# FordyceLab/magnify

Measured on NVIDIA B200. Metric: roi_pixels_per_sec, higher is better.
Workload: dtype u16

## Files before the change

### include/magnify_b200.h

```cpp
#ifndef MAGNIFY_B200_H
#define MAGNIFY_B200_H

#include <stdint.h>

#ifdef __cplusplus
extern "C" {
#endif

#define MGB_ABI_VERSION 12

#define MGB_OK 0
#define MGB_EINVAL (-1)
#define MGB_EALIGN (-2)
#define MGB_EUNSUPPORTED (-3)
#define MGB_EIO (-4)
#define MGB_EFORMAT (-5)

#define MGB_U8 0
#define MGB_U16 1
#define MGB_F32 2
#define MGB_F64 3

int mgb_abi_version(void);
const char* mgb_error_string(int code);
// ... 23 lines not shown
                             const double* bias, const double* maxima, void* stream);
int mgb_flatfield_apply_generic(const void* tiles, void* out, int dtype, int64_t C, int64_t P,
                                int64_t HW, int K, const double* flat, const double* dark,
                                const double* maxima, void* stream);

int mgb_copy2d_async(void* dst, int64_t dst_pitch_bytes, const void* src, int64_t src_pitch_bytes,
                     int64_t width_bytes, int64_t rows, int kind, void* stream);

int mgb_bounding_boxes(const double* x, const double* y, int64_t n, int L, int64_t W, int64_t H,
                       int32_t* boxes, int32_t* rel, void* stream);

int mgb_set_tma_enabled(int enabled);
int mgb_set_gather_loader(int loader);

int mgb_roi_gather(const void* image, int64_t image_pitch, int64_t C, int64_t T, int64_t H, int64_t W,
                   int itemsize, const int32_t* boxes, const int32_t* order, int64_t M, int L, void* roi,
                   void* stream);
int mgb_roi_gather_stats_u16(const uint16_t* image, int64_t image_pitch, int64_t C, int64_t T, int64_t H,
                             int64_t W, const int32_t* boxes, const int32_t* order, const int32_t* mask_t,
                             int64_t Tm, const uint8_t* fg, const uint8_t* bg, int64_t M, int L,
                             uint16_t* roi, double* stats, int want_median, int fg_count_max,
                             int bg_count_max, int* host_median_done, void* stream);
int mgb_mask_count_max(const uint8_t* fg, const uint8_t* bg, int64_t n_masks, int64_t mask_len,
                       int32_t* counts, void* stream);
int mgb_roi_gather_stats_peers_u16(const uint16_t* image, int64_t image_pitch, int64_t C, int64_t T,
                                   int64_t H, int64_t W, const int32_t* boxes, const int32_t* order, const int32_t* mask_t,
                                   int64_t Tm, const uint8_t* fg, const uint8_t* bg, int64_t M, int L,
                                   uint16_t* roi, const uint64_t* host_peer_stats, int n_peers,
                                   int want_median, int fg_count_max, int bg_count_max,
                                   int* host_median_done, void* stream);
int mgb_roi_stats_u16(const uint16_t* roi, int64_t M, int64_t C, int64_t T, int L,
                      const int32_t* mask_t, int64_t Tm, const uint8_t* fg, const uint8_t* bg,
                      double* stats, void* stream);
int mgb_roi_median_u16(const uint16_t* roi, int64_t M, int64_t C, int64_t T, int L,
                       const int32_t* mask_t, int64_t Tm, const uint8_t* mask, double* median,
                       int64_t median_stride, void* stream);

int mgb_roi_stats_f32(const float* roi, int64_t M, int64_t C, int64_t T, int L, const int32_t* mask_t, int64_t Tm,
                      const uint8_t* fg, const uint8_t* bg, double* stats, void* stream);
int mgb_roi_median_f32(const float* roi, int64_t M, int64_t C, int64_t T, int L, const int32_t* mask_t, int64_t Tm,
                       const uint8_t* mask, double* median, int64_t median_stride, void* stream);

int mgb_chip_masks(const int32_t* rel, const int32_t* r_fg, int r_inner, int r_outer, int64_t M,
                   int L, uint8_t* fg, uint8_t* bg, int32_t* counts, void* stream);

int mgb_mask_perimeters(const uint8_t* masks, int64_t M, int L, double* perimeter, void* stream);

int mgb_disc_halfwidths(int r, int32_t* host_hw);
int mgb_bead_labels(const int32_t* beads, int64_t M, int64_t H, int64_t W, const int32_t* hw,
                    int rmax, int32_t* labels, void* stream);
int mgb_bead_masks(const int32_t* labels, int64_t H, int64_t W, const int32_t* boxes, int64_t M,
                   int L, uint8_t* fg, uint8_t* bg, int32_t* counts, void* stream);

int mgb_to_uint8(const void* src, int dtype, int64_t B, int64_t n, uint8_t* dst, double* minmax, void* stream);
int mgb_edge_gradients_u8(const uint8_t* image, int64_t B, int64_t H, int64_t W, uint8_t* blurred, int16_t* dx,
                          int16_t* dy, void* stream);
int mgb_gradient_order_stats(const int16_t* dx, const int16_t* dy, int64_t B, int64_t n, const int64_t* host_ranks,
                             int n_ranks, int64_t* host_values, uint32_t* scratch, void* stream);
int mgb_canny(const int16_t* dx, const int16_t* dy, int64_t B, int64_t H, int64_t W, const int32_t* thresholds,
              uint8_t* edges, int* changed, int* host_sweeps, void* stream);

int mgb_edge_cell_lists(const uint8_t* edges, int64_t B, int64_t H, int64_t W, int grid_length, int64_t* counts,
                        int64_t* starts, uint32_t* coords, int64_t coords_capacity, int64_t* host_total, void* stream);
int mgb_sample_circles(const uint32_t* coords, const int64_t* starts, const int64_t* counts, int64_t B, int64_t H,
                       int64_t W, int grid_length, int64_t num_iter, float min_radius, float max_radius,
                       uint64_t seed, const uint32_t* randoms, float* raw, uint64_t* table, int64_t table_capacity,
// ... 30 lines not shown
```

### magnify_b200/_lib.py

```python
from __future__ import annotations

import ctypes
import os
from ctypes import c_char_p, c_int, c_int64, c_void_p, POINTER

_PKG_DIR = os.path.dirname(os.path.abspath(__file__))
LIB_PATH = os.path.join(_PKG_DIR, "libmagnify_b200.so")

MGB_U8, MGB_U16, MGB_F32, MGB_F64 = 0, 1, 2, 3
MGB_EINVAL, MGB_EALIGN, MGB_EUNSUPPORTED, MGB_EIO, MGB_EFORMAT = -1, -2, -3, -4, -5


class MagnifyB200Error(RuntimeError):
    def __init__(self, fn: str, code: int, text: str):
        super().__init__(f"{fn} failed with status {code}: {text}")
        self.fn, self.code = fn, code


_P = c_void_p
_I64 = c_int64
SIGNATURES = {
    "mgb_abi_version": [],
    "mgb_error_string": [c_int],
    "mgb_sm_count": [],
    "mgb_launch_count": [],
    "mgb_l2_persist": [_P, _P, _I64, ctypes.c_float],
    "mgb_set_tma_enabled": [c_int],
    "mgb_set_stitch_variant": [c_int],
    "mgb_set_gather_loader": [c_int],
    "mgb_stitch": [_P, _P, _I64, _I64, _I64, _I64, _I64, _I64, _I64, _I64, c_int, POINTER(c_int), _P],
    "mgb_flatfield_tilemax_u16": [_P, _I64, _I64, _I64, c_int, c_int, _P, _P],
    "mgb_flatfield_maxima": [_P, c_int, c_int, _I64, _P, _P, _P, _P],
    "mgb_flatfield_maxima_generic": [_P, c_int, _I64, _I64, _I64, c_int, _P, _P, _P, _P],
    "mgb_flatfield_tables": [_P, _P, c_int, _I64, _P, _P, _P, _P],
    "mgb_flatfield_stitch_u16": [_P, _P, _I64, _I64, _I64, _I64, _I64, _I64, _I64, _I64, c_int, _P, _P, _P, _P, _P, _P],
    "mgb_flatfield_apply_generic": [_P, _P, c_int, _I64, _I64, _I64, c_int, _P, _P, _P, _P],
    "mgb_copy2d_async": [_P, _I64, _P, _I64, _I64, _I64, c_int, _P],
    "mgb_bounding_boxes": [_P, _P, _I64, c_int, _I64, _I64, _P, _P, _P],
    "mgb_roi_gather": [_P, _I64, _I64, _I64, _I64, _I64, c_int, _P, _P, _I64, c_int, _P, _P],
    "mgb_roi_gather_stats_u16": [_P, _I64, _I64, _I64, _I64, _I64, _P, _P, _P, _I64, _P, _P, _I64, c_int, _P, _P,
                                 c_int, c_int, c_int, POINTER(c_int), _P],
    "mgb_mask_count_max": [_P, _P, _I64, _I64, _P, _P],
    "mgb_roi_gather_stats_peers_u16": [_P, _I64, _I64, _I64, _I64, _I64, _P, _P, _P, _I64, _P, _P, _I64, c_int, _P,
                                       POINTER(ctypes.c_uint64), c_int, c_int, c_int, c_int, POINTER(c_int), _P],
    "mgb_roi_stats_u16": [_P, _I64, _I64, _I64, c_int, _P, _I64, _P, _P, _P, _P],
    "mgb_roi_median_u16": [_P, _I64, _I64, _I64, c_int, _P, _I64, _P, _P, _I64, _P],
    "mgb_roi_stats_f32": [_P, _I64, _I64, _I64, c_int, _P, _I64, _P, _P, _P, _P],
    "mgb_roi_median_f32": [_P, _I64, _I64, _I64, c_int, _P, _I64, _P, _P, _I64, _P],
    "mgb_chip_masks": [_P, _P, c_int, c_int, _I64, c_int, _P, _P, _P, _P],
    "mgb_disc_halfwidths": [c_int, POINTER(ctypes.c_int32)],
    "mgb_bead_labels": [_P, _I64, _I64, _I64, _P, c_int, _P, _P],
    "mgb_bead_masks": [_P, _I64, _I64, _P, _I64, c_int, _P, _P, _P, _P],
    "mgb_mask_perimeters": [_P, _I64, c_int, _P, _P],
    "mgb_to_uint8": [_P, c_int, _I64, _I64, _P, _P, _P],
    "mgb_edge_gradients_u8": [_P, _I64, _I64, _I64, _P, _P, _P, _P],
    "mgb_gradient_order_stats": [_P, _P, _I64, _I64, POINTER(c_int64), c_int, POINTER(c_int64), _P, _P],
    "mgb_canny": [_P, _P, _I64, _I64, _I64, _P, _P, _P, POINTER(c_int), _P],
    "mgb_edge_cell_lists": [_P, _I64, _I64, _I64, c_int, _P, _P, _P, _I64, POINTER(c_int64), _P],
    "mgb_sample_circles": [_P, _P, _P, _I64, _I64, _I64, c_int, _I64, ctypes.c_float, ctypes.c_float, ctypes.c_uint64,
                           _P, _P, _P, _I64, _P, POINTER(c_int64), _P, _P],
    "mgb_gradient_angles": [_P, _P, _P, _I64, _P, _P],
    "mgb_circle_perimeter": [c_int, c_int, POINTER(ctypes.c_int32), c_int, POINTER(c_int)],
    "mgb_score_circles": [_P, _I64, _I64, _I64, _P, _P, c_int, c_int, _P, _P, _P, _P, _P],
    "mgb_order_circles": [_P, _P, _I64, _P, _P],
    "mgb_filter_neighbors_device": [_P, _I64, _I64, _I64, _I64, c_int, c_int, _P, _P, POINTER(c_int), _P],
    "mgb_filter_neighbors": [POINTER(ctypes.c_int32), _I64, c_int, POINTER(ctypes.c_uint8)],
    "mgb_tiff_open": [c_char_p, POINTER(c_void_p)],
    "mgb_tiff_close": [_P],
    "mgb_tiff_page_count": [_P, POINTER(c_int64)],
    "mgb_tiff_page_info": [_P, _I64, POINTER(c_int64)],
    "mgb_tiff_description": [_P, _I64, c_char_p, _I64],
    "mgb_tiff_read_pages": [_P, POINTER(c_int64), _I64, _P, _I64, c_int],
    "mgb_tiff_write": [c_char_p, _P, _I64, _I64, _I64, c_int, c_int, c_int, c_char_p, c_int],
    "mgb_tiff_read_files": [POINTER(c_char_p), _I64, _I64, _I64, _I64, c_int, _P, _I64, c_int],
}
_SPECIAL_RESTYPE = {"mgb_error_string": c_char_p, "mgb_launch_count": c_int64}
_NO_STATUS = {"mgb_abi_version", "mgb_error_string", "mgb_sm_count", "mgb_launch_count", "mgb_set_tma_enabled", "mgb_set_stitch_variant", "mgb_set_gather_loader"}

# ... 38 lines not shown
```

### magnify_b200/csrc/roi.cu

```cuda
#include "common.cuh"

namespace mgb {

__device__ __forceinline__ void box_1d(long long c, int L, long long size, long long* lo) {
  long long a = c - L / 2;
  long long b = c + (L + 1) / 2;
  if (a < 0) { b -= a; a = 0; }
  if (b > size) { a -= b - size; }
  *lo = a;
}

__global__ void __launch_bounds__(kThreads)
bounding_boxes_kernel(const double* __restrict__ x, const double* __restrict__ y, int64_t n, int L,
                      int64_t W, int64_t H, int32_t* __restrict__ boxes, int32_t* __restrict__ rel) {
  const int64_t i = (int64_t)blockIdx.x * blockDim.x + threadIdx.x;
  if (i >= n) return;
  const long long xr = __double2ll_rn(x[i]);
  const long long yr = __double2ll_rn(y[i]);
  long long top, left;
  box_1d(yr, L, H, &top);
  box_1d(xr, L, W, &left);
  boxes[2 * i] = (int32_t)top;
  boxes[2 * i + 1] = (int32_t)left;
  if (rel) {
// ... 312 lines not shown
    const float x = src[i];
    if (x != x) continue;
    if (fg[moff + i]) { v[0] += 1.0; v[2] += (double)x; }
    if (bg[moff + i]) { v[1] += 1.0; v[3] += (double)x; }
  }
#pragma unroll
  for (int k = 0; k < 4; ++k) {
    for (int o = 16; o > 0; o >>= 1) v[k] += __shfl_down_sync(0xffffffffu, v[k], o);
    if ((threadIdx.x & 31) == 0) red[k][threadIdx.x >> 5] = v[k];
  }
  __syncthreads();
  if (threadIdx.x == 0) {
    double s[4] = {0.0, 0.0, 0.0, 0.0};
    for (int w = 0; w < kThreads / 32; ++w)
      for (int k = 0; k < 4; ++k) s[k] += red[k][w];
    double* out = stats + n * kRec;
    out[0] = s[0]; out[1] = s[1]; out[2] = s[2]; out[3] = s[3];
    out[4] = s[2] / s[0];
    out[5] = s[3] / s[1];
    out[6] = out[7] = __longlong_as_double(0x7ff8000000000000LL);
  }
}

static uint32_t magic_for(uint32_t d) { return (uint32_t)((0x100000000ULL + d - 1) / d); }

int roi_gather_tma(const void* image, int64_t pitch, int64_t C, int64_t T, int64_t H, int64_t W, int itemsize,
                   const int32_t* boxes, const int32_t* order, const int32_t* mask_t, int64_t Tm, const uint8_t* fg,
                   const uint8_t* bg, int64_t M, int L, void* roi, double* stats, const uint64_t* host_peers,
                   int n_peers, cudaStream_t st);

int roi_gather_lists(const void* image, int64_t pitch, int64_t C, int64_t T, int64_t H, int64_t W,
                     const int32_t* boxes, const int32_t* order, const int32_t* mask_t, int64_t Tm, const uint8_t* fg,
                     const uint8_t* bg, int64_t M, int L, void* roi, double* stats, int want_median, int nf_max,
                     int nb_max, const uint64_t* host_peers, int n_peers, cudaStream_t st);

extern int g_gather_loader;
extern int g_gather_wpm;

static int g_tma_enabled = 1;

}

using namespace mgb;

template <typename TPix>
static int launch_roi_median(const TPix* roi, int64_t M, int64_t C, int64_t T, int L, const int32_t* mask_t, int64_t Tm,
                             const uint8_t* mask, double* median, int64_t stride, void* stream) {
  if (M < 0 || C < 0 || T < 0 || L <= 0 || stride < 1) return MGB_EINVAL;
  const int64_t n_roi = M * C * T;
  if (n_roi == 0) return MGB_OK;
  if (n_roi > INT32_MAX) return MGB_EUNSUPPORTED;
  if (!roi || !mask_t || !mask || !median || Tm <= 0) return MGB_EINVAL;
  cudaStream_t st = (cudaStream_t)stream;
  const int npt = (int)ceil_div((int64_t)L * L, kThreads);
#define MGB_MED(N) roi_median_kernel<N, TPix><<<(unsigned)n_roi, kThreads, 0, st>>>(roi, C, T, L, mask_t, Tm, mask, median, stride)
  if (npt <= 4) MGB_MED(4);
  else if (npt <= 10) MGB_MED(10);
  else if (npt <= 21) MGB_MED(21);
  else if (npt <= 40) MGB_MED(40);
  else if (npt <= 64) MGB_MED(64);
  else if (npt <= 100) MGB_MED(100);
  else roi_median_big_kernel<TPix><<<(unsigned)n_roi, kThreads, 0, st>>>(roi, C, T, L, mask_t, Tm, mask, median, stride);
#undef MGB_MED
  MGB_CUDA_LAUNCH_CHECK();
  return MGB_OK;
}

// ... 94 lines not shown
}

int mgb_roi_gather_stats_u16(const uint16_t* image, int64_t image_pitch, int64_t C, int64_t T, int64_t H,
                             int64_t W, const int32_t* boxes, const int32_t* order, const int32_t* mask_t, int64_t Tm,
                             const uint8_t* fg, const uint8_t* bg, int64_t M, int L,
                             uint16_t* roi, double* stats, int want_median, int fg_count_max, int bg_count_max,
                             int* host_median_done, void* stream) {
  if (host_median_done) *host_median_done = 0;
  if (!stats && M * C * T > 0) return MGB_EINVAL;
  return gather_common(image, image_pitch, C, T, H, W, 2, boxes, order, 0, mask_t, Tm, fg, bg, M, L, roi, stats,
                       (cudaStream_t)stream, nullptr, 0, want_median, fg_count_max, bg_count_max, host_median_done);
}

int mgb_roi_gather_stats_peers_u16(const uint16_t* image, int64_t image_pitch, int64_t C, int64_t T, int64_t H,
                                   int64_t W, const int32_t* boxes, const int32_t* order, const int32_t* mask_t,
                                   int64_t Tm, const uint8_t* fg, const uint8_t* bg, int64_t M, int L,
                                   uint16_t* roi, const uint64_t* host_peer_stats, int n_peers, int want_median,
                                   int fg_count_max, int bg_count_max, int* host_median_done, void* stream) {
  if (host_median_done) *host_median_done = 0;
  if (!host_peer_stats || n_peers < 1 || n_peers > 8) return MGB_EINVAL;
  if (M * C * T == 0) return MGB_OK;
  return gather_common(image, image_pitch, C, T, H, W, 2, boxes, order, 0, mask_t, Tm, fg, bg, M, L, roi,
                       reinterpret_cast<double*>(host_peer_stats[0]), (cudaStream_t)stream, host_peer_stats, n_peers,
                       want_median, fg_count_max, bg_count_max, host_median_done);
}

int mgb_roi_stats_u16(const uint16_t* roi, int64_t M, int64_t C, int64_t T, int L, const int32_t* mask_t,
                      int64_t Tm, const uint8_t* fg, const uint8_t* bg, double* stats, void* stream) {
  if (!stats && M * C * T > 0) return MGB_EINVAL;
  return gather_common(roi, 0, C, T, L, L, 2, nullptr, nullptr, C * T * (int64_t)L * L, mask_t, Tm, fg, bg, M, L, nullptr,
                       stats, (cudaStream_t)stream);
}

int mgb_roi_median_u16(const uint16_t* roi, int64_t M, int64_t C, int64_t T, int L,
                       const int32_t* mask_t, int64_t Tm, const uint8_t* mask, double* median,
                       int64_t median_stride, void* stream) {
  return launch_roi_median<uint16_t>(roi, M, C, T, L, mask_t, Tm, mask, median, median_stride, stream);
}

int mgb_roi_median_f32(const float* roi, int64_t M, int64_t C, int64_t T, int L, const int32_t* mask_t, int64_t Tm,
                       const uint8_t* mask, double* median, int64_t median_stride, void* stream) {
  return launch_roi_median<float>(roi, M, C, T, L, mask_t, Tm, mask, median, median_stride, stream);
}

int mgb_roi_stats_f32(const float* roi, int64_t M, int64_t C, int64_t T, int L, const int32_t* mask_t, int64_t Tm,
                      const uint8_t* fg, const uint8_t* bg, double* stats, void* stream) {
  if (M < 0 || C < 0 || T < 0 || L <= 0) return MGB_EINVAL;
  const int64_t n_roi = M * C * T;
  if (n_roi == 0) return MGB_OK;
  if (n_roi > INT32_MAX) return MGB_EUNSUPPORTED;
  if (!roi || !mask_t || !fg || !bg || !stats || Tm <= 0) return MGB_EINVAL;
  roi_stats_f32_kernel<<<(unsigned)n_roi, kThreads, 0, (cudaStream_t)stream>>>(roi, C, T, L, mask_t, Tm, fg, bg, stats);
  MGB_CUDA_LAUNCH_CHECK();
  return MGB_OK;
}

}
```

### magnify_b200/csrc/roi_lists.cu

```cuda
#include <algorithm>

#include "roi_stage.cuh"

namespace mgb {

constexpr int kNFL = 32;
constexpr int kNBL = 80;

__device__ __forceinline__ void stage_mask(const uint8_t* __restrict__ g, int n, uint8_t* s, int tid, int nth) {
  const uint32_t sa = smem_u32(s);
  if ((reinterpret_cast<uintptr_t>(g) & 15u) == 0) {
    const int nv = n >> 4;
    for (int i = tid; i < nv; i += nth)
      asm volatile("cp.async.ca.shared.global [%0], [%1], 16;" ::"r"(sa + 16u * i), "l"(g + 16 * i) : "memory");
    for (int i = (nv << 4) + tid; i < n; i += nth) s[i] = g[i];
  } else if ((reinterpret_cast<uintptr_t>(g) & 3u) == 0) {
    const int nv = n >> 2;
    for (int i = tid; i < nv; i += nth)
      asm volatile("cp.async.ca.shared.global [%0], [%1], 4;" ::"r"(sa + 4u * i), "l"(g + 4 * i) : "memory");
    for (int i = (nv << 2) + tid; i < n; i += nth) s[i] = g[i];
  } else {
    for (int i = tid; i < n; i += nth) s[i] = g[i];
  }
}
// ... 217 lines not shown
  const bool overflow = nf > (uint32_t)p.cap_f || nb > (uint32_t)p.cap_b;
  if (active && !overflow) {
    pad_list(fl, nf, p.cap_f, WPM ? lane : (int)threadIdx.x, WPM ? 32 : (int)blockDim.x);
    pad_list(bl, nb, p.cap_b, WPM ? lane : (int)threadIdx.x, WPM ? 32 : (int)blockDim.x);
  }
  __syncthreads();
  if (!active) return;
  const double cnt_fg = (double)nf, cnt_bg = (double)nb;
  const int GF = p.cap_f >> 8, GB = p.cap_b >> 8;
  const uint32_t pad_f = (uint32_t)p.cap_f - nf, pad_b = (uint32_t)p.cap_b - nb;

  const int nt = s_nt;
  const int n_items = nt * (int)p.C;

  constexpr int kV = VPL > 0 ? VPL : 1;
  const int nquads = (p.rows * p.wu) >> 2;

  uint8_t* my_stages = stages + (size_t)warp * p.n_stages * p.stage_bytes;
  const uint32_t my_stage0 = smem_u32(my_stages);
  const uint32_t my_bar0 = smem_u32(&bars[warp * 4]);
  uint32_t* my_hist = hists + (size_t)warp * kHistWords;
  const uint32_t tx_bytes = (uint32_t)(p.rows * p.wpu * 2);
  const int first = WPM ? 0 : part * nw + warp, step = WPM ? 1 : nparts * nw;

  struct Cursor { int i, c, k; };
  auto advance = [&](Cursor& cur, int by) {
    cur.i += by;
    cur.k += by;
    while (cur.k >= nt) { cur.k -= nt; ++cur.c; }
  };
  auto issue_tma = [&](const Cursor& cur, int s) {
    if (lane == 0) {
      const int64_t t = tlist[cur.k];
      const int32_t top = p.boxes[(m * p.T + t) * 2];
      const int32_t left = p.boxes[(m * p.T + t) * 2 + 1];
      const uint32_t bar = my_bar0 + s * 8;
      mbar_expect_tx(bar, tx_bytes);
      tma_load_3d(my_stage0 + s * p.stage_bytes, &tmap, bar, left & ~7, top, (int)(cur.c * p.T + t));
    }
  };

  Cursor ahead{0, 0, 0}, cur{0, 0, 0};
  if (nt > 0) { advance(ahead, first); advance(cur, first); }
  for (int s = 0; s < p.n_stages; ++s) {
    if (ahead.i < n_items) issue_tma(ahead, s);
    if (nt > 0) advance(ahead, step);
  }
  int s = 0;
  uint32_t parity = 0;
  for (; cur.i < n_items; advance(cur, step)) {
    const int64_t c = cur.c, t = tlist[cur.k];
    const int shift = p.boxes[(m * p.T + t) * 2 + 1] & 7;
    const int64_t n = (m * p.C + c) * p.T + t;
    const uint8_t* buf = my_stages + (size_t)s * p.stage_bytes;
    mbar_wait(my_bar0 + s * 8, parity);

    if (p.store) {
      uint16_t* dst = p.roi + n * (int64_t)p.rows * p.wu;
      uint32_t opaque = 0;
      asm volatile("" : "+r"(opaque));
      if constexpr (QPL > 0) {
        uint2* d2 = reinterpret_cast<uint2*>(dst);
        const uint32_t* s32 = reinterpret_cast<const uint32_t*>(buf);
        auto copy = [&](auto par) {
          constexpr int PAR = decltype(par)::value;
#pragma unroll
          for (int k = 0; k < QPL; ++k) {
            const int q = lane + 32 * k;
            if (q < nquads) {
              const uint32_t u = 4u * q + opaque;
              const uint32_t row = __umulhi(u, p.magic_wu), col = u - row * p.wu;
              const uint32_t oa = row * p.wpu + col + shift;
              const uint32_t ob = (col + 2 < (uint32_t)p.wu) ? oa + 2 : (row + 1) * p.wpu + shift;
              const uint32_t lo = load_pair<PAR>(s32, oa);
              const uint32_t hi = load_pair<PAR>(s32, ob);
              asm volatile("st.global.L1::no_allocate.v2.u32 [%0], {%1,%2};" ::"l"(d2 + q), "r"(lo), "r"(hi) : "memory");
            }
          }
        };
        if (shift & 1) copy(std::integral_constant<int, 1>{});
        else copy(std::integral_constant<int, 0>{});
      } else {
        uint32_t dummy_f, dummy_b;
        if (p.vpr) {
          uint32_t svo[kV];
// ... 73 lines not shown
    if (++s == p.n_stages) { s = 0; parity ^= 1; }
  }
}

__global__ void __launch_bounds__(kThreads)
mask_count_max_kernel(const uint8_t* __restrict__ fg, const uint8_t* __restrict__ bg, int64_t n_masks, int64_t len,
                      int32_t* __restrict__ out) {
  const int64_t w = ((int64_t)blockIdx.x * blockDim.x + threadIdx.x) >> 5;
  const int lane = threadIdx.x & 31;
  if (w >= n_masks) return;
  const uint8_t* f = fg + w * len;
  const uint8_t* b = bg + w * len;
  uint32_t cf = 0, cb = 0;
  for (int64_t i = lane; i < len; i += 32) {
    cf += f[i] != 0;
    cb += b[i] != 0;
  }
  cf = __reduce_add_sync(0xffffffffu, cf);
  cb = __reduce_add_sync(0xffffffffu, cb);
  if (lane == 0) {
    atomicMax(out, (int32_t)cf);
    atomicMax(out + 1, (int32_t)cb);
  }
}

PFN_cuTensorMapEncodeTiled get_encode_fn();
extern int g_gather_wpm;

static uint32_t magic_u32_(uint32_t d) { return (uint32_t)((0x100000000ULL + d - 1) / d); }

int roi_gather_lists(const void* image, int64_t pitch, int64_t C, int64_t T, int64_t H, int64_t W,
                     const int32_t* boxes, const int32_t* order, const int32_t* mask_t, int64_t Tm, const uint8_t* fg,
                     const uint8_t* bg, int64_t M, int L, void* roi, double* stats, int want_median, int nf_max,
                     int nb_max, const uint64_t* host_peers, int n_peers, cudaStream_t st) {
  if (!stats || nf_max < 0 || nb_max < 0) return MGB_EALIGN;
  if (nf_max > kNFL * 32 || nb_max > kNBL * 32) return MGB_EALIGN;
  const int wu = L;
  const int wpu = (wu + 7 + 7) & ~7;
  if ((pitch * 2) % 16 != 0 || !aligned16(image) || wpu > 256 || L > 256) return MGB_EALIGN;
  if ((int64_t)(L - 1) * wpu + L + 8 > 65535) return MGB_EALIGN;
  if (C * T > INT32_MAX || H > INT32_MAX || pitch > INT32_MAX || M > INT32_MAX || Tm > 65535) return MGB_EALIGN;
  PFN_cuTensorMapEncodeTiled encode = get_encode_fn();
  if (!encode) return MGB_EALIGN;

  TmaGatherParams p{};
  p.roi = (uint16_t*)roi; p.boxes = boxes; p.order = order; p.mask_t = mask_t; p.fg = fg; p.bg = bg; p.stats = stats;
  p.C = C; p.T = T; p.Tm = Tm; p.rows = L; p.wu = wu; p.wpu = wpu; p.unit = 1;
  p.n_peers = 0;
  if (host_peers && n_peers > 0) {
    if (n_peers > 8) return MGB_EINVAL;
    p.n_peers = n_peers;
    for (int j = 0; j < n_peers; ++j) p.peer_stats[j] = reinterpret_cast<double*>(host_peers[j]);
  }
  p.stage_bytes = (L * wpu * 2 + 127) & ~127;
  p.cap_f = (std::max(nf_max, 1) + 255) & ~255;
  p.cap_b = (std::max(nb_max, 1) + 255) & ~255;
  p.want_median = want_median ? 1 : 0;
  p.store = roi ? 1 : 0;
  const bool out16 = !roi || aligned16(roi);
  const bool out8 = !roi || (reinterpret_cast<uintptr_t>(roi) & 7u) == 0;
  const bool out4 = !roi || (reinterpret_cast<uintptr_t>(roi) & 3u) == 0;
  int vpl = 0, qpl = 0;
  if (wu % 8 == 0 && wu > 8 && out16) {
    p.vpr = (uint32_t)(wu / 8);
    p.magic_vpr = magic_u32_(p.vpr);
    const int v = (int)((L * p.vpr + 31) / 32);
    vpl = v <= 12 ? 12 : v <= 21 ? 21 : v <= 36 ? 36 : 0;
  } else if (wu % 2 == 0 && (L * wu) % 4 == 0 && out8 && (L * wu / 4 + 31) / 32 <= 24) {
    qpl = (L * wu / 4 + 31) / 32 <= 12 ? 12 : 24;
  } else if (wu % 2 == 0 && wu > 2 && out4) {
    p.half = (uint32_t)(wu / 2);
    p.magic_half = magic_u32_(p.half);
  }

  const int64_t items = C * std::max<int64_t>(1, T / std::max<int64_t>(1, Tm));
  int dev = 0, max_smem = 0, sms = 0;
  MGB_CUDA_TRY(cudaGetDevice(&dev));
  MGB_CUDA_TRY(cudaDeviceGetAttribute(&max_smem, cudaDevAttrMaxSharedMemoryPerBlockOptin, dev));
  MGB_CUDA_TRY(cudaDeviceGetAttribute(&sms, cudaDevAttrMultiProcessorCount, dev));
  bool wpm = g_gather_wpm && items < 128 && M * Tm >= (int64_t)sms * 12 * 8;
  if (const char* e = getenv("MGB_GATHER_LAYOUT")) wpm = atoi(e) == 1 ? true : atoi(e) == 0 ? false : wpm;

  const size_t list_bytes = (size_t)(p.cap_f + p.cap_b) * sizeof(uint16_t);
  int sm_smem = 0;
  MGB_CUDA_TRY(cudaDeviceGetAttribute(&sm_smem, cudaDevAttrMaxSharedMemoryPerMultiprocessor, dev));
  int nw = 0, ns = 0;
  size_t smem_bytes = 0;
  int want_nw = 0;
  if (const char* e = getenv("MGB_GATHER_WARPS")) want_nw = atoi(e);
  for (int pass = 0; pass < 2 && !nw; ++pass) {
    const bool pair = !wpm && items < 128;
    for (int cand : {6, 16, 12, 8, 4}) {
      if (want_nw ? cand != want_nw : ((cand == 6 && !pair) || (cand == 16 && !wpm))) continue;
      const size_t fixed = (wpm ? cand : 1) * list_bytes + (size_t)cand * kHistWords * sizeof(uint32_t) +
                           (size_t)cand * 4 * sizeof(uint64_t) + (size_t)T * sizeof(int32_t) + 128;
      const size_t room = cand == 6 ? (size_t)(sm_smem / 2 - 1024) : (size_t)max_smem;
      if (room < fixed + 1024) continue;
      const bool one = cand >= 12 || cand == 6;
      const int n = (int)std::min<size_t>(one ? 1 : 4, (room - fixed - 1024) / ((size_t)cand * p.stage_bytes));
      if (n >= (one ? 1 : 2)) { nw = cand; ns = n; smem_bytes = (size_t)cand * n * p.stage_bytes + fixed; break; }
    }
    if (!nw && wpm) wpm = false;
  }
  if (!nw) return MGB_EALIGN;
  bool split_tail = true;
  if (const char* e = getenv("MGB_GATHER_SPLIT")) split_tail = atoi(e) != 0;
  p.n_stages = ns;
  p.magic_wu = magic_u32_((uint32_t)wu);

  CUtensorMap tmap;
  const cuuint64_t gdim[3] = {(cuuint64_t)pitch, (cuuint64_t)H, (cuuint64_t)(C * T)};
  const cuuint64_t gstride[2] = {(cuuint64_t)pitch * 2, (cuuint64_t)H * pitch * 2};
  const cuuint32_t box[3] = {(cuuint32_t)wpu, (cuuint32_t)L, 1};
  const cuuint32_t estr[3] = {1, 1, 1};
  const CUresult cr = encode(&tmap, CU_TENSOR_MAP_DATA_TYPE_UINT16, 3, const_cast<void*>(image), gdim, gstride, box,
                             estr, CU_TENSOR_MAP_INTERLEAVE_NONE, CU_TENSOR_MAP_SWIZZLE_NONE,
                             CU_TENSOR_MAP_L2_PROMOTION_NONE, CU_TENSOR_MAP_FLOAT_OOB_FILL_NONE);
  if (cr != CUDA_SUCCESS) return MGB_EALIGN;
  p.image = (const uint16_t*)image;
  p.H = H;
  p.Wu = pitch;

  const uint32_t magic_l = magic_u32_((uint32_t)L);
#define MGB_LAUNCH_L(VP, QP, WP, NWARPS)                                                                   \
  do {                                                                                                    \
    auto kern = roi_gather_lists_kernel<VP, QP, WP, NWARPS>;                                              \
    MGB_CUDA_TRY(cudaFuncSetAttribute(kern, cudaFuncAttributeMaxDynamicSharedMemorySize, (int)smem_bytes)); \
    dim3 grid(WP ? (unsigned)((M + nw - 1) / nw) : (unsigned)M, (unsigned)Tm);                            \
    p.split_from = M;                                                                                     \
    p.split_parts = 1;                                                                                    \
    if (!WP && split_tail) {                                                                          \
      int resident = 1;                                                                                   \
      MGB_CUDA_TRY(cudaOccupancyMaxActiveBlocksPerMultiprocessor(&resident, kern, nw * 32, smem_bytes));  \
      const int64_t slots = (int64_t)std::max(resident, 1) * sms, tail = (M * Tm) % slots;                \
      const int64_t rounds = (items + nw - 1) / nw;                                                       \
      const int parts = (int)std::min<int64_t>({8, tail ? slots / tail : 1, rounds});                     \
      if (Tm == 1 && M > slots && parts >= 2) {                                                           \
        p.split_from = M - tail;                                                                          \
        p.split_parts = parts;                                                                            \
        grid.x = (unsigned)(p.split_from + tail * parts);                                                 \
      }                                                                                                   \
    }                                                                                                     \
    kern<<<grid, nw * 32, smem_bytes, st>>>(tmap, p, M, magic_l);                                         \
  } while (0)
#define MGB_LAUNCH_NW(VP, QP, WP)                       \
  do {                                                  \
    if (nw == 16) MGB_LAUNCH_L(VP, QP, WP, 16);         \
    else if (nw == 12) MGB_LAUNCH_L(VP, QP, WP, 12);    \
    else if (nw == 6) MGB_LAUNCH_L(VP, QP, WP, 6);      \
    else MGB_LAUNCH_L(VP, QP, WP, 8);                   \
  } while (0)
// ... 36 lines not shown
```

### magnify_b200/csrc/roi_stage.cuh

```cuda
#pragma once
#include <cstdlib>
#include <type_traits>

#include <cuda.h>
#include <cudaTypedefs.h>

#include "common.cuh"

namespace mgb {

constexpr int kTmaMaxWarps = 8;

struct TmaGatherParams {
  uint16_t* roi;
  const int32_t* boxes;
  const int32_t* order;
  const int32_t* mask_t;
  const uint8_t* fg;
  const uint8_t* bg;
  double* stats;
  double* peer_stats[8];
  int n_peers;
  int64_t C, T, Tm;
  int rows;
  int wu;
  int wpu;
  int unit;
  int n_stages;
  int loader;
  const uint16_t* image;
  int64_t H, Wu;
  int stage_bytes;
  uint32_t vpr;
  uint32_t magic_vpr;
  uint32_t half;
  uint32_t magic_half;
  uint32_t magic_wu;
  int cap_f, cap_b;
  int want_median;
  int store;
  int split_parts;
  int64_t split_from;
};

__device__ __forceinline__ uint32_t smem_u32(const void* p) {
  return (uint32_t)__cvta_generic_to_shared(p);
}
__device__ __forceinline__ void mbar_init(uint32_t bar, uint32_t count) {
  asm volatile("mbarrier.init.shared::cta.b64 [%0], %1;" ::"r"(bar), "r"(count) : "memory");
}
__device__ __forceinline__ void mbar_expect_tx(uint32_t bar, uint32_t bytes) {
  asm volatile("mbarrier.arrive.expect_tx.shared::cta.b64 _, [%0], %1;" ::"r"(bar), "r"(bytes) : "memory");
}
__device__ __forceinline__ void mbar_wait(uint32_t bar, uint32_t parity) {
  uint32_t done = 0;
  while (!done) {
    asm volatile(
        "{\n"
        ".reg .pred p;\n"
        "mbarrier.try_wait.parity.shared::cta.b64 p, [%1], %2;\n"
        "selp.u32 %0, 1, 0, p;\n"
        "}\n"
        : "=r"(done)
        : "r"(bar), "r"(parity)
        : "memory");
  }
}
__device__ __forceinline__ void tma_load_3d(uint32_t dst, const CUtensorMap* map, uint32_t bar, int c0,
                                            int c1, int c2) {
  asm volatile(
      "cp.async.bulk.tensor.3d.shared::cluster.global.mbarrier::complete_tx::bytes "
      "[%0], [%1, {%3, %4, %5}], [%2];" ::"r"(dst), "l"(map), "r"(bar), "r"(c0), "r"(c1), "r"(c2)
      : "memory");
}

template <int S>
__device__ __forceinline__ uint4 shift_units(const uint4& a, const uint4& b) {
  const uint32_t w[8] = {a.x, a.y, a.z, a.w, b.x, b.y, b.z, b.w};
  constexpr int o = S >> 1;
  if constexpr ((S & 1) == 0) {
    return make_uint4(w[o], w[o + 1], w[o + 2], w[o + 3]);
  } else {
    return make_uint4(__funnelshift_r(w[o], w[o + 1], 16), __funnelshift_r(w[o + 1], w[o + 2], 16),
                      __funnelshift_r(w[o + 2], w[o + 3], 16), __funnelshift_r(w[o + 3], w[o + 4], 16));
  }
}

constexpr int kStatsRec = 8;
__device__ __forceinline__ double nan_f64() { return __longlong_as_double(0x7ff8000000000000LL); }
__device__ __forceinline__ void write_stats(const TmaGatherParams& p, int lane, int64_t n, double cf, double cb,
                                            double sf, double sb, double mf, double mb) {
  double* o = nullptr;
  if (p.n_peers == 0) {
    if (lane == 0) o = p.stats + n * kStatsRec;
  } else if (lane < p.n_peers) {
    o = p.peer_stats[lane] + n * kStatsRec;
  }
  if (o) {
    double2* o2 = reinterpret_cast<double2*>(o);
    o2[0] = make_double2(cf, cb);
    o2[1] = make_double2(sf, sb);
    o2[2] = make_double2(sf / cf, sb / cb);
    o2[3] = make_double2(mf, mb);
  }
}

// ... 107 lines not shown
```

### magnify_b200/ops.py

```python
from __future__ import annotations

import ctypes
from typing import Optional, Sequence

import numpy as np
import torch

from . import _lib

STATS = ("n_fg", "n_bg", "sum_fg", "sum_bg", "mean_fg", "mean_bg", "median_fg", "median_bg")
NSTATS = len(STATS)

_DTYPE_CODE = {
    torch.uint8: _lib.MGB_U8,
    torch.uint16: _lib.MGB_U16,
    torch.float32: _lib.MGB_F32,
    torch.float64: _lib.MGB_F64,
}


_UNSIGNED = (torch.uint8, torch.uint16)


def _stream() -> ctypes.c_void_p:
# ... 417 lines not shown
    done = ctypes.c_int(0)
    if peer_stats is not None:
        n_peers = len(peer_stats)
        arr = (ctypes.c_uint64 * n_peers)(*[int(a) for a in peer_stats])
        with torch.cuda.device(image.device):
            _lib.call("mgb_roi_gather_stats_peers_u16", _ptr(image), pitch, c, t, h, w, _ptr(boxes),
                      _ptr(_check_order(order, m)), _ptr(mask_t), tm, _ptr(fg), _ptr(bg), m, int(roi_length),
                      _ptr(roi), arr, n_peers, int(bool(medians)), nf_max, nb_max, ctypes.byref(done), _stream())
        if medians and not done.value and m * c * t > 0:
            raise RuntimeError("peer_stats needs the fused gather (masks of at most 1024 fg / 2560 bg pixels per marker, "
                               "uint16 image); gather locally and all_gather the summaries instead")
        return roi, None
    with torch.cuda.device(image.device):
        _lib.call("mgb_roi_gather_stats_u16", _ptr(image), pitch, c, t, h, w, _ptr(boxes), _ptr(_check_order(order, m)),
                  _ptr(mask_t), tm, _ptr(fg), _ptr(bg), m, int(roi_length), _ptr(roi), _ptr(stats),
                  int(bool(medians)), nf_max, nb_max, ctypes.byref(done), _stream())
    global last_gather_fused
    last_gather_fused = bool(done.value) or not medians
    if medians and not done.value and m * c * t > 0:
        crops = roi if roi is not None else roi_gather(image, boxes, roi_length, order=order)
        _median_into(crops, fg, mask_t, tm, stats, 6)
        _median_into(crops, bg, mask_t, tm, stats, 7)
    return roi, stats


def _median_into(roi, mask, mask_t, tm, stats, column: int) -> None:
    m, c, t, length, _ = roi.shape
    out = stats.view(-1)[column:]
    with torch.cuda.device(roi.device):
        _lib.call("mgb_roi_median_u16" if roi.dtype == torch.uint16 else "mgb_roi_median_f32", _ptr(roi), m, c, t,
                  int(length), _ptr(mask_t), tm, _ptr(mask), _ptr(out), NSTATS, _stream())


def roi_stats(roi: torch.Tensor, fg: torch.Tensor, bg: torch.Tensor, mask_t: Optional[torch.Tensor] = None,
              medians: bool = True) -> torch.Tensor:
    if roi.dtype not in (torch.uint16, torch.float32):
        raise TypeError(f"roi must be uint16 or float32, got {roi.dtype}")
    _check(roi, "roi", ndim=5)
    m, c, t, length, _ = roi.shape
    fg, bg, tm = _masks_u8(fg, bg, m, length)
    mask_t = _default_mask_t(mask_t, tm, t, roi.device)
    stats = torch.empty((m, c, t, NSTATS), dtype=torch.float64, device=roi.device)
    with torch.cuda.device(roi.device):
        _lib.call("mgb_roi_stats_u16" if roi.dtype == torch.uint16 else "mgb_roi_stats_f32", _ptr(roi), m, c, t,
                  int(length), _ptr(mask_t), tm, _ptr(fg), _ptr(bg), _ptr(stats), _stream())
    if medians and m * c * t > 0:
        _median_into(roi, fg, mask_t, tm, stats, 6)
        _median_into(roi, bg, mask_t, tm, stats, 7)
    return stats


def roi_median(roi: torch.Tensor, mask: torch.Tensor, mask_t: Optional[torch.Tensor] = None) -> torch.Tensor:
    if roi.dtype not in (torch.uint16, torch.float32):
        raise TypeError(f"roi must be uint16 or float32, got {roi.dtype}")
    _check(roi, "roi", ndim=5)
    m, c, t, length, _ = roi.shape
    mask = mask.view(torch.uint8) if mask.dtype == torch.bool else mask
    _check(mask, "mask", dtype=torch.uint8, ndim=4)
    tm = mask.shape[1]
    if tuple(mask.shape) != (m, tm, length, length):
        raise ValueError(f"mask must have shape ({m}, Tm, {length}, {length})")
    mask_t = _default_mask_t(mask_t, tm, t, roi.device, "mask")
    out = torch.empty((m, c, t), dtype=torch.float64, device=roi.device)
    with torch.cuda.device(roi.device):
        _lib.call("mgb_roi_median_u16" if roi.dtype == torch.uint16 else "mgb_roi_median_f32", _ptr(roi), m, c, t,
                  int(length), _ptr(mask_t), tm, _ptr(mask), _ptr(out), 1, _stream())
    return out


def chip_masks(rel: torch.Tensor, fg_radius: torch.Tensor, inner_radius: int, outer_radius: int, roi_length: int,
               want_counts: bool = False):
    _check(rel, "rel", dtype=torch.int32, ndim=2)
    _check(fg_radius, "fg_radius", dtype=torch.int32, ndim=1)
    m = rel.shape[0]
    if rel.shape[1] != 2 or fg_radius.shape[0] != m:
# ... 84 lines not shown
```

Measured before the change: 132.6 billion.

## Route u16 roi_stats through fused list-based stats kernel with bulk crop loads

Adds a crops mode to the TMA list-gather stats kernel: instead of tensor-map loads from the image, it issues 1D bulk async copies of contiguous pre-gathered crops into shared memory. roi_stats for uint16 now uses this kernel, which computes sums, means and medians in one pass, replacing the separate stats kernel plus two median kernels. The cost targeted is the three launches and the repeated reads of the ROI tensor. It adds a mask_count_max call when counts are not supplied, and it falls back to the old path when alignment checks fail.

```diff
diff --git a/include/magnify_b200.h b/include/magnify_b200.h
--- a/include/magnify_b200.h
+++ b/include/magnify_b200.h
@@ -79,6 +79,9 @@
 int mgb_roi_stats_u16(const uint16_t* roi, int64_t M, int64_t C, int64_t T, int L,
                       const int32_t* mask_t, int64_t Tm, const uint8_t* fg, const uint8_t* bg,
                       double* stats, void* stream);
+int mgb_roi_stats_lists_u16(const uint16_t* roi, int64_t M, int64_t C, int64_t T, int L, const int32_t* order,
+                            const int32_t* mask_t, int64_t Tm, const uint8_t* fg, const uint8_t* bg, double* stats,
+                            int want_median, int fg_count_max, int bg_count_max, void* stream);
 int mgb_roi_median_u16(const uint16_t* roi, int64_t M, int64_t C, int64_t T, int L,
                        const int32_t* mask_t, int64_t Tm, const uint8_t* mask, double* median,
                        int64_t median_stride, void* stream);
diff --git a/magnify_b200/_lib.py b/magnify_b200/_lib.py
--- a/magnify_b200/_lib.py
+++ b/magnify_b200/_lib.py
@@ -44,6 +44,7 @@
     "mgb_roi_gather_stats_peers_u16": [_P, _I64, _I64, _I64, _I64, _I64, _P, _P, _P, _I64, _P, _P, _I64, c_int, _P,
                                        POINTER(ctypes.c_uint64), c_int, c_int, c_int, c_int, POINTER(c_int), _P],
     "mgb_roi_stats_u16": [_P, _I64, _I64, _I64, c_int, _P, _I64, _P, _P, _P, _P],
+    "mgb_roi_stats_lists_u16": [_P, _I64, _I64, _I64, c_int, _P, _P, _I64, _P, _P, _P, c_int, c_int, c_int, _P],
     "mgb_roi_median_u16": [_P, _I64, _I64, _I64, c_int, _P, _I64, _P, _P, _I64, _P],
     "mgb_roi_stats_f32": [_P, _I64, _I64, _I64, c_int, _P, _I64, _P, _P, _P, _P],
     "mgb_roi_median_f32": [_P, _I64, _I64, _I64, c_int, _P, _I64, _P, _P, _I64, _P],
diff --git a/magnify_b200/csrc/roi.cu b/magnify_b200/csrc/roi.cu
--- a/magnify_b200/csrc/roi.cu
+++ b/magnify_b200/csrc/roi.cu
@@ -368,7 +368,8 @@
 int roi_gather_lists(const void* image, int64_t pitch, int64_t C, int64_t T, int64_t H, int64_t W,
                      const int32_t* boxes, const int32_t* order, const int32_t* mask_t, int64_t Tm, const uint8_t* fg,
                      const uint8_t* bg, int64_t M, int L, void* roi, double* stats, int want_median, int nf_max,
-                     int nb_max, const uint64_t* host_peers, int n_peers, cudaStream_t st);
+                     int nb_max, const uint64_t* host_peers, int n_peers, cudaStream_t st,
+                     const uint16_t* crops = nullptr);
 
 extern int g_gather_loader;
 extern int g_gather_wpm;
@@ -529,6 +530,17 @@
                        stats, (cudaStream_t)stream);
 }
 
+int mgb_roi_stats_lists_u16(const uint16_t* roi, int64_t M, int64_t C, int64_t T, int L, const int32_t* order,
+                            const int32_t* mask_t, int64_t Tm, const uint8_t* fg, const uint8_t* bg, double* stats,
+                            int want_median, int fg_count_max, int bg_count_max, void* stream) {
+  if (M < 0 || C < 0 || T < 0 || L <= 0) return MGB_EINVAL;
+  if (M * C * T == 0) return MGB_OK;
+  if (M * C * T > INT32_MAX) return MGB_EUNSUPPORTED;
+  if (!roi || !mask_t || !fg || !bg || !stats || Tm <= 0) return MGB_EINVAL;
+  return roi_gather_lists(nullptr, L, C, T, L, L, nullptr, order, mask_t, Tm, fg, bg, M, L, nullptr, stats,
+                          want_median, fg_count_max, bg_count_max, nullptr, 0, (cudaStream_t)stream, roi);
+}
+
 int mgb_roi_median_u16(const uint16_t* roi, int64_t M, int64_t C, int64_t T, int L,
                        const int32_t* mask_t, int64_t Tm, const uint8_t* mask, double* median,
                        int64_t median_stride, void* stream) {
diff --git a/magnify_b200/csrc/roi_lists.cu b/magnify_b200/csrc/roi_lists.cu
--- a/magnify_b200/csrc/roi_lists.cu
+++ b/magnify_b200/csrc/roi_lists.cu
@@ -273,11 +273,16 @@
   auto issue_tma = [&](const Cursor& cur, int s) {
     if (lane == 0) {
       const int64_t t = tlist[cur.k];
-      const int32_t top = p.boxes[(m * p.T + t) * 2];
-      const int32_t left = p.boxes[(m * p.T + t) * 2 + 1];
       const uint32_t bar = my_bar0 + s * 8;
       mbar_expect_tx(bar, tx_bytes);
-      tma_load_3d(my_stage0 + s * p.stage_bytes, &tmap, bar, left & ~7, top, (int)(cur.c * p.T + t));
+      if (p.crops) {
+        const int64_t n = (m * p.C + cur.c) * p.T + t;
+        bulk_load_1d(my_stage0 + s * p.stage_bytes, p.crops + n * (int64_t)p.rows * p.rows, tx_bytes, bar);
+      } else {
+        const int32_t top = p.boxes[(m * p.T + t) * 2];
+        const int32_t left = p.boxes[(m * p.T + t) * 2 + 1];
+        tma_load_3d(my_stage0 + s * p.stage_bytes, &tmap, bar, left & ~7, top, (int)(cur.c * p.T + t));
+      }
     }
   };
 
@@ -291,7 +296,7 @@
   uint32_t parity = 0;
   for (; cur.i < n_items; advance(cur, step)) {
     const int64_t c = cur.c, t = tlist[cur.k];
-    const int shift = p.boxes[(m * p.T + t) * 2 + 1] & 7;
+    const int shift = p.crops ? 0 : p.boxes[(m * p.T + t) * 2 + 1] & 7;
     const int64_t n = (m * p.C + c) * p.T + t;
     const uint8_t* buf = my_stages + (size_t)s * p.stage_bytes;
     mbar_wait(my_bar0 + s * 8, parity);
@@ -431,18 +436,24 @@
 int roi_gather_lists(const void* image, int64_t pitch, int64_t C, int64_t T, int64_t H, int64_t W,
                      const int32_t* boxes, const int32_t* order, const int32_t* mask_t, int64_t Tm, const uint8_t* fg,
                      const uint8_t* bg, int64_t M, int L, void* roi, double* stats, int want_median, int nf_max,
-                     int nb_max, const uint64_t* host_peers, int n_peers, cudaStream_t st) {
+                     int nb_max, const uint64_t* host_peers, int n_peers, cudaStream_t st,
+                     const uint16_t* crops) {
   if (!stats || nf_max < 0 || nb_max < 0) return MGB_EALIGN;
   if (nf_max > kNFL * 32 || nb_max > kNBL * 32) return MGB_EALIGN;
   const int wu = L;
-  const int wpu = (wu + 7 + 7) & ~7;
-  if ((pitch * 2) % 16 != 0 || !aligned16(image) || wpu > 256 || L > 256) return MGB_EALIGN;
+  const int wpu = crops ? L : (wu + 7 + 7) & ~7;
+  if (crops) {
+    if (roi || L % 4 != 0 || !aligned16(crops) || L > 256) return MGB_EALIGN;
+  } else if ((pitch * 2) % 16 != 0 || !aligned16(image) || wpu > 256 || L > 256) {
+    return MGB_EALIGN;
+  }
   if ((int64_t)(L - 1) * wpu + L + 8 > 65535) return MGB_EALIGN;
   if (C * T > INT32_MAX || H > INT32_MAX || pitch > INT32_MAX || M > INT32_MAX || Tm > 65535) return MGB_EALIGN;
   PFN_cuTensorMapEncodeTiled encode = get_encode_fn();
-  if (!encode) return MGB_EALIGN;
+  if (!crops && !encode) return MGB_EALIGN;
 
   TmaGatherParams p{};
+  p.crops = crops;
   p.roi = (uint16_t*)roi; p.boxes = boxes; p.order = order; p.mask_t = mask_t; p.fg = fg; p.bg = bg; p.stats = stats;
   p.C = C; p.T = T; p.Tm = Tm; p.rows = L; p.wu = wu; p.wpu = wpu; p.unit = 1;
   p.n_peers = 0;
@@ -507,15 +518,17 @@
   p.n_stages = ns;
   p.magic_wu = magic_u32_((uint32_t)wu);
 
-  CUtensorMap tmap;
-  const cuuint64_t gdim[3] = {(cuuint64_t)pitch, (cuuint64_t)H, (cuuint64_t)(C * T)};
-  const cuuint64_t gstride[2] = {(cuuint64_t)pitch * 2, (cuuint64_t)H * pitch * 2};
-  const cuuint32_t box[3] = {(cuuint32_t)wpu, (cuuint32_t)L, 1};
-  const cuuint32_t estr[3] = {1, 1, 1};
-  const CUresult cr = encode(&tmap, CU_TENSOR_MAP_DATA_TYPE_UINT16, 3, const_cast<void*>(image), gdim, gstride, box,
-                             estr, CU_TENSOR_MAP_INTERLEAVE_NONE, CU_TENSOR_MAP_SWIZZLE_NONE,
-                             CU_TENSOR_MAP_L2_PROMOTION_NONE, CU_TENSOR_MAP_FLOAT_OOB_FILL_NONE);
-  if (cr != CUDA_SUCCESS) return MGB_EALIGN;
+  CUtensorMap tmap{};
+  if (!crops) {
+    const cuuint64_t gdim[3] = {(cuuint64_t)pitch, (cuuint64_t)H, (cuuint64_t)(C * T)};
+    const cuuint64_t gstride[2] = {(cuuint64_t)pitch * 2, (cuuint64_t)H * pitch * 2};
+    const cuuint32_t box[3] = {(cuuint32_t)wpu, (cuuint32_t)L, 1};
+    const cuuint32_t estr[3] = {1, 1, 1};
+    const CUresult cr = encode(&tmap, CU_TENSOR_MAP_DATA_TYPE_UINT16, 3, const_cast<void*>(image), gdim, gstride, box,
+                               estr, CU_TENSOR_MAP_INTERLEAVE_NONE, CU_TENSOR_MAP_SWIZZLE_NONE,
+                               CU_TENSOR_MAP_L2_PROMOTION_NONE, CU_TENSOR_MAP_FLOAT_OOB_FILL_NONE);
+    if (cr != CUDA_SUCCESS) return MGB_EALIGN;
+  }
   p.image = (const uint16_t*)image;
   p.H = H;
   p.Wu = pitch;
diff --git a/magnify_b200/csrc/roi_stage.cuh b/magnify_b200/csrc/roi_stage.cuh
--- a/magnify_b200/csrc/roi_stage.cuh
+++ b/magnify_b200/csrc/roi_stage.cuh
@@ -41,6 +41,7 @@
   int store;
   int split_parts;
   int64_t split_from;
+  const uint16_t* crops;
 };
 
 __device__ __forceinline__ uint32_t smem_u32(const void* p) {
@@ -72,6 +73,11 @@
       "cp.async.bulk.tensor.3d.shared::cluster.global.mbarrier::complete_tx::bytes "
       "[%0], [%1, {%3, %4, %5}], [%2];" ::"r"(dst), "l"(map), "r"(bar), "r"(c0), "r"(c1), "r"(c2)
       : "memory");
+}
+__device__ __forceinline__ void bulk_load_1d(uint32_t dst, const void* src, uint32_t bytes, uint32_t bar) {
+  asm volatile("cp.async.bulk.shared::cluster.global.mbarrier::complete_tx::bytes [%0], [%1], %2, [%3];"
+               ::"r"(dst), "l"(src), "r"(bytes), "r"(bar)
+               : "memory");
 }
 
 template <int S>
diff --git a/magnify_b200/ops.py b/magnify_b200/ops.py
--- a/magnify_b200/ops.py
+++ b/magnify_b200/ops.py
@@ -473,8 +473,12 @@
                   int(length), _ptr(mask_t), tm, _ptr(mask), _ptr(out), NSTATS, _stream())
 
 
+last_stats_fused = True
+
+
 def roi_stats(roi: torch.Tensor, fg: torch.Tensor, bg: torch.Tensor, mask_t: Optional[torch.Tensor] = None,
-              medians: bool = True) -> torch.Tensor:
+              medians: bool = True, order: Optional[torch.Tensor] = None,
+              mask_counts: Optional[Sequence[int]] = None) -> torch.Tensor:
     if roi.dtype not in (torch.uint16, torch.float32):
         raise TypeError(f"roi must be uint16 or float32, got {roi.dtype}")
     _check(roi, "roi", ndim=5)
@@ -482,6 +486,20 @@
     fg, bg, tm = _masks_u8(fg, bg, m, length)
     mask_t = _default_mask_t(mask_t, tm, t, roi.device)
     stats = torch.empty((m, c, t, NSTATS), dtype=torch.float64, device=roi.device)
+    global last_stats_fused
+    last_stats_fused = False
+    if roi.dtype == torch.uint16 and length % 4 == 0 and roi.data_ptr() % 16 == 0 and m * c * t > 0:
+        if mask_counts is None:
+            mask_counts = mask_count_max(fg, bg) if m * tm > 0 else (0, 0)
+        with torch.cuda.device(roi.device):
+            rc = _lib.try_call("mgb_roi_stats_lists_u16", _ptr(roi), m, c, t, int(length),
+                               _ptr(_check_order(order, m)), _ptr(mask_t), tm, _ptr(fg), _ptr(bg), _ptr(stats),
+                               int(bool(medians)), int(mask_counts[0]), int(mask_counts[1]), _stream())
+        if rc == 0:
+            last_stats_fused = True
+            return stats
+        if rc != _lib.MGB_EALIGN:
+            raise _lib.MagnifyB200Error("mgb_roi_stats_lists_u16", rc, _lib.error_string(rc))
     with torch.cuda.device(roi.device):
         _lib.call("mgb_roi_stats_u16" if roi.dtype == torch.uint16 else "mgb_roi_stats_f32", _ptr(roi), m, c, t,
                   int(length), _ptr(mask_t), tm, _ptr(fg), _ptr(bg), _ptr(stats), _stream())
```

Measured after the change: 132.6 billion, median of 6. About the same (-0.1%).
